# pdrebello/flash-attention-minitorch

Measured on AMD Instinct MI355X. Metric: attn fw+bw TFLOP/s at (B=8,H=8,N=4096,d=64); % MFMA roofline, higher is better.
Workload: dtype bf16

## Files before the change

flash_attention_minitorch_amd/csrc/fa_api.hip:

```cpp
#include <hip/hip_runtime.h>
#include <math.h>
#include <algorithm>
#include <chrono>
#include <mutex>
#include <string>
#include <vector>
#include <stdio.h>
#include <stdlib.h>
#include <string.h>
#include <unistd.h>
#include <atomic>

#include "../../include/flash_attn_mi355x.h"
#include "fa_kernels.h"

namespace {

thread_local char g_err[512] = "";

int set_err(int code, const char* what, hipError_t e = hipSuccess) {
  if (e != hipSuccess)
    snprintf(g_err, sizeof(g_err), "%s: %s", what, hipGetErrorString(e));
  else
    snprintf(g_err, sizeof(g_err), "%s", what);
  return code;
}

#define FA_HIP_TRY(expr)                                             \
  do {                                                               \
    hipError_t e_ = (expr);                                          \
    if (e_ != hipSuccess) return set_err(FA_ERR_HIP, #expr, e_);     \
  } while (0)

constexpr double FWD_SPLITK_MAX_WGS_PER_CU = 0.5, FWD_SPLITK_MAX_WGS_PER_CU_CAUSAL = 1.0;

inline bool d_supported(int d) { return d == 32 || d == 64 || d == 128; }
inline int d_padded(int d) { return d <= 32 ? 32 : (d <= 64 ? 64 : 128); }

constexpr int NTUN = 10;
struct Tun { int v[NTUN]; };
inline Tun default_tun() { return Tun{{0, 0, 0, 0, 0, 0, 0, 0, 0, 0}}; }
int parse_opts(const int* opts, int nopts, Tun& t) {
  t = default_tun();
  if (nopts < 0 || nopts > NTUN || (nopts > 0 && !opts)) return set_err(FA_ERR_BAD_ARG, "bad options array");
  for (int i = 0; i < nopts; ++i) t.v[i] = opts[i];
  static const int allowed[NTUN][7] = {{0, 3, 4, 5, 6, 7, -1}, {0, 2, 3, 4, -1}, {0, 2, 3, -1}, {0, -1}, {0, 1, 4, 5, -1}, {0, 1, -1}, {0, -1}, {0, 1, 2, -1},
                                       {0, 1, 2, 3, -1}, {0, 1, -1}};
  for (int i = 0; i < NTUN; ++i) {
    bool ok = false;
    for (int j = 0; allowed[i][j] >= 0; ++j) ok |= allowed[i][j] == t.v[i];
    if (!ok) return set_err(FA_ERR_BAD_ARG, "option value not supported (retired diagnostic values included)");
  }
  return FA_OK;
}

constexpr int WS_VECS = 3;

struct Call {
  const void *q = nullptr, *k = nullptr, *v = nullptr, *dout = nullptr;
  float *out = nullptr, *l = nullptr, *m = nullptr, *dq = nullptr, *dk = nullptr, *dv = nullptr, *ws = nullptr;
  bool bwd = false;
  int B = 0, H = 1;
  bool by_heads = false;
  int layout = FA_LAYOUT_BHND;
  int N = 0, d = 0;
  bool padded = false;
  int dp = 0;
  int causal = 0, variant = 0, dtype = 0;
  int stages = 0;
  const int* opts = nullptr;
  int nopts = 0;
  const float* kmask = nullptr;
  int mask_heads = 1;
  float drop_rate = 0.f, drop_scale = 1.f;
  unsigned drop_seed = 0;
  float scale = 0.f;
  bool scale_required = false;
  const float* guard = nullptr;
  int produce = 0;
  bool gqa = false;
  int Hkv = 0;
  float *gdk = nullptr, *gdv = nullptr;
  hipStream_t st = nullptr;
  int batch = 0;
  Tun tun = default_tun();
  fa::Layout lay{};
  float tau = 0.f;
  float* nlc() const { return ws; }
  float* delta() const { return ws + (long)batch * N; }
  float* nl2() const { return ws + 2 * (long)batch * N; }
};

int device_cus_raw();
int device_cus() {
  const int n = device_cus_raw();
  return n > 0 ? n : 256;
}
int device_cus_raw() {
  static std::mutex mu;
  static int cus[64];
  int dev = 0;
  if (hipGetDevice(&dev) != hipSuccess || dev < 0 || dev >= 64) return 0;
  std::lock_guard<std::mutex> lock(mu);
  if (cus[dev] == 0) {
    int n = 0;
    if (hipDeviceGetAttribute(&n, hipDeviceAttributeMultiprocessorCount, dev) != hipSuccess) return 0;
    cus[dev] = n;
  }
  return cus[dev];
}

int rank_chunk(int wgs_per_cu, int nb) {
  return std::max(1, device_cus() * wgs_per_cu / (4 * nb));
}

bool causal_ranked(const Tun& tun, int blocks, int wgs_per_cu) {
  if (tun.v[7]) return tun.v[7] == 2;
  return blocks < 8 * device_cus() * wgs_per_cu;
}

int head_tiles(const Call& c, int nb) {
  int tiles = 1;
  if (c.N % 256 == 0 && c.tun.v[5] == 0 && c.lay.G == 1) {
    const int cus = device_cus();
    for (int t = 2; t <= 16; ++t)
      if (c.batch % t == 0 && (c.batch / t) % 8 == 0 && (long)(c.batch / t) * nb >= cus) tiles = t;
  }
  return tiles;
}

inline bool guard_rows_fold(int dtype, int row_elems) { return dtype == FA_DTYPE_BF16 && (row_elems == 64 || row_elems == 128); }
int launch_scale_guard(const void* q, const void* k, long rows, long krows, int row_elems, int dtype, void* guard, hipStream_t st) {
  if (!guard_rows_fold(dtype, row_elems)) {
    FA_HIP_TRY(hipMemsetAsync(guard, 0, (size_t)2 * fa::GUARD_SLOTS * sizeof(float), st));
    return FA_OK;
  }
  const dim3 grid(fa::GUARD_SLOTS, 2);
  if (row_elems == 64)
    hipLaunchKernelGGL((fa::scale_guard_kernel<64>), grid, dim3(256), 0, st, (const fa::bf16_t*)q, (const fa::bf16_t*)k, rows, krows, (float*)guard);
  else
    hipLaunchKernelGGL((fa::scale_guard_kernel<128>), grid, dim3(256), 0, st, (const fa::bf16_t*)q, (const fa::bf16_t*)k, rows, krows, (float*)guard);
  FA_HIP_TRY(hipGetLastError());
  return FA_OK;
}

#define FA_KERNS(X)                                                                                                                  \
  X(FWD_SPLITK, "fwd_splitk_f32_kernel")                                                                                             \
  X(FWD_SLOT_CAUSAL, "fwd_slot_kernel") X(FWD_SLOT_WHOLE, "fwd_slot_kernel") X(FWD_SLOT_MASKED, "fwd_slot_kernel")                   \
  X(FWD_DROP, "fwd_kernel") X(FWD_MASK, "fwd_kernel") X(FWD_CARE, "fwd_kernel") X(FWD_MAIN, "fwd_kernel")                            \
  X(BWD_PREP, "bwd_prep_kernel")                                                                                                     \
  X(DQ_DROP, "bwd_dq_kernel") X(DQ_MASK, "bwd_dq_kernel") X(DQ_CARE, "bwd_dq_kernel") X(DQ_MAIN, "bwd_dq_kernel")                    \
  X(DQ_WAVE8, "bwd_dq_kernel")                                                                                                       \
  X(DQ_SLOT_CAUSAL, "bwd_dq_slot_kernel") X(DQ_SLOT_TILED, "bwd_dq_slot_kernel") X(DQ_SLOT_WHOLE, "bwd_dq_slot_kernel")              \
  X(DQ_SLOT_MASKED, "bwd_dq_slot_kernel")                                                                                            \
  X(DKDV_SLOT, "bwd_dkdv_slot_kernel") X(DKDV_SLOT_CAUSAL, "bwd_dkdv_slot_kernel")                                                   \
  X(DKDV_SLOT64_TILED, "bwd_dkdv_slot_kernel")            \
  X(DKDV_CARE_DROP, "bwd_dkdv_kernel") X(DKDV_CARE, "bwd_dkdv_kernel") X(DKDV_DROP_F32, "bwd_dkdv_kernel")                           \
  X(DKDV_CARE_MAIN, "bwd_dkdv_kernel") X(DKDV_PAIRED, "bwd_dkdv_kernel") X(DKDV_PAIRED_M3, "bwd_dkdv_kernel")                        \
  X(DKDV_PLAIN, "bwd_dkdv_kernel") X(DKDV_F32_64, "bwd_dkdv_kernel")                                                                 \
  X(ONEPASS, "bwd_onepass_f32_kernel")                                                                                               \
  X(GROUP_SUM, "group_sum_kernel")          \
  X(GUARD_PASS, "scale_guard_kernel")                                                        \
  X(GUARD_PASS_ZERO, nullptr)                             \
  X(GUARD_ZERO, "memset")                                                  \
  X(ZERO_GRADS, nullptr)
#define X(id, name) id,
enum Kern : int { FA_KERNS(X) };
#undef X
#define X(id, name) name,
constexpr const char* KERN_NAME[] = {FA_KERNS(X)};
#undef X
#define X(id, name) #id,
constexpr const char* BUILD_NAME[] = {FA_KERNS(X)};
#undef X

struct Step {
  Kern kern;
  unsigned grid, block;
  int nb;
  int arg;
  int rank_chunk = 0, tiles = 0, twin_blocks = 0, guard_want = 0;
  bool prep = false;
  bool check = true;
};
struct Selection {
  Step steps[8] = {};
  int n = 0;
  bool folds = false;
  bool produces_guard = false;
  bool fuses_prep = false;
  int onepass = 0;
  Step& add(Kern kern, int grid, int block, int nb = 0, int arg = 0) {
    return steps[n++] = Step{kern, (unsigned)grid, (unsigned)block, nb, arg};
  }
  void append(const Selection& o, int guard_want = 0) {
    for (int i = 0; i < o.n; ++i) (steps[n++] = o.steps[i]).guard_want = guard_want;
    folds |= o.folds;
    produces_guard |= o.produces_guard;
    fuses_prep |= o.fuses_prep;
    onepass |= o.onepass;
  }
};

void select_phased(Selection& s, const Call& c, bool bf, Kern base, int only_qb, int care_main, int ranked, bool prep) {
  const int batch = c.batch, N = c.N, causal = c.causal, nqb = (N + 127) / 128;
  const bool fwd = base == FWD_DROP;
  const int chunk = (ranked && causal && only_qb < 0) ? rank_chunk(2, nqb) : 0;
  int twin = 1;
  if (fwd && c.lay.guard && c.lay.guard_want == 1 && !causal && only_qb < 0)
    for (int t = 4; t > 1; t >>= 1)
      if (nqb % t == 0 && (long)batch * (nqb / t) >= 2L * device_cus()) { twin = t; break; }
  const int nblk = only_qb >= 0 ? 1 : ((causal && !chunk) ? (nqb + 1) / 2 : nqb / twin);
  const int build = c.lay.drop_thr ? 0
                    : c.lay.kmask  ? 1
                    : (bf && (N < 64 || only_qb >= 0 || (causal && care_main))) ? 2 : 3;
  Step& m = s.add(Kern(base + build), batch * nblk, 256, nqb, only_qb);
  m.rank_chunk = chunk;
  m.twin_blocks = fwd ? twin : 0;
  if (build != 3) return;
  m.prep = prep;
  if (bf && causal) {
    m.check = false;
    s.add(Kern(base + 2), batch, 256, nqb, 0).twin_blocks = m.twin_blocks;
  }
}

template <typename T, int D>
Selection select_fwd(const Call& c) {
  constexpr bool BF = sizeof(T) == 2;
  const int batch = c.batch, N = c.N, causal = c.causal;
  const Tun& tun = c.tun;
  const bool plain = !c.lay.kmask && !c.lay.drop_thr;
  Selection s;
  if (!BF && D == 64) {
    const long wgs = (long)batch * ((N + 127) / 128), cus = device_cus();
    if (plain && !c.lay.out_bf16 && N >= 128 && (tun.v[1] == 4 ||
         (tun.v[1] == 0 && wgs <= (causal ? FWD_SPLITK_MAX_WGS_PER_CU_CAUSAL : FWD_SPLITK_MAX_WGS_PER_CU) * cus))) {
      const int nqb = (N + 31) / 32;
      s.add(FWD_SPLITK, batch * nqb, 256, nqb);
      return s;
    }
  }
  if (BF && (D == 64 || D == 128)) {
    const int nqb = (N + 255) / 256;
    const bool cslot = causal && N % 256 == 0 && (tun.v[1] == 3 || (tun.v[1] == 0 && batch * nqb >= 256));
    if (c.variant == FA_VARIANT_FA2 && tun.v[1] != 2 && (!causal || tun.v[1] == 3 || cslot) && plain && N >= 64) {
      if (cslot) {
        const bool ranked = causal_ranked(tun, batch * nqb, D == 64 ? 2 : 1);
        s.add(FWD_SLOT_CAUSAL, ranked ? batch * nqb : batch * ((nqb + 1) / 2), 512, nqb, ranked ? 2 : 1).rank_chunk =
            rank_chunk(D == 64 ? 2 : 1, nqb);
        s.folds = true;
        return s;
      }
      if (!causal && N % (8192 / D) == 0) {
        s.add(FWD_SLOT_WHOLE, batch * nqb, 512, nqb, causal);
        s.folds = s.produces_guard = true;
        return s;
      }
      if (D == 64) {
        s.add(FWD_SLOT_MASKED, batch * nqb, 512, nqb, causal);
        if (causal) select_phased(s, c, BF, FWD_DROP, 0, 0, 0, false);
        return s;
      }
    }
  }
  select_phased(s, c, BF, FWD_DROP, -1, D == 64 ? 1 : 0, tun.v[7] == 2 || (tun.v[7] == 0 && BF && D == 32), false);
  return s;
}

template <typename T, int D>
void select_dkdv_phased(Selection& s, const Call& c, bool mode3 = false, int care_main = 0, int rank_causal = 1) {
  constexpr bool BF = sizeof(T) == 2;
  constexpr int NW = BF ? 8 : 4;
  const int batch = c.batch, N = c.N, causal = c.causal;
  const int nkb = (N + NW * 32 - 1) / (NW * 32), nkb4 = (N + 127) / 128;
  const bool rank = causal && rank_causal;
  if (c.lay.drop_thr) {
    if (BF) s.add(DKDV_CARE_DROP, batch * nkb4, 256, nkb4).rank_chunk = rank ? rank_chunk(2, nkb4) : 0;
    else s.add(DKDV_DROP_F32, batch * nkb, NW * 64, nkb).rank_chunk = rank ? rank_chunk(2, nkb) : 0;
    return;
  }
  if (BF && (c.lay.kmask || N < 64)) {
    s.add(DKDV_CARE, batch * nkb4, 256, nkb4).rank_chunk = rank ? rank_chunk(2, nkb4) : 0;
    return;
  }
  if (mode3 && causal && care_main) {
    s.add(DKDV_CARE_MAIN, batch * ((nkb + 1) / 2), NW * 64, nkb);
    return;
  }
  const int thin = (BF && causal) ? 1 : 0;
  Step* m;
  if ((causal || mode3) && !(BF && D == 128)) {
    m = &s.add(mode3 ? DKDV_PAIRED_M3 : DKDV_PAIRED, batch * ((nkb + 1) / 2), NW * 64, nkb, thin);
  } else {
    m = &s.add(DKDV_PLAIN, batch * nkb, NW * 64, nkb, thin);
    m->rank_chunk = rank ? rank_chunk(NW == 8 ? 1 : 2, nkb) : 0;
  }
  if (thin) {
    m->check = false;
    s.add(DKDV_CARE, batch, 256, nkb4, 2).rank_chunk = m->rank_chunk;
  }
}

template <typename T, int D>
int onepass_f32(const Call& c) {
  const int N = c.N;
  const Tun& tun = c.tun;
  const int both = FA_BWD_STAGE_DKDV | FA_BWD_STAGE_DQ;
  if (!(sizeof(T) == 4 && D == 64 && (c.stages & both) == both && (tun.v[4] == 0 || tun.v[4] == 5) && !c.lay.kmask &&
        !c.lay.drop_thr && N >= 256))
    return 0;
  static const bool deterministic = [] { const char* e = getenv("FA_MI355X_DETERMINISTIC"); return e && e[0] == '1'; }();
  if (deterministic && tun.v[4] != 5) return 0;
  const long cus = device_cus(), wgs1 = (long)c.batch * ((N + 255) / 256), nqi = (N + 31) / 32;
  for (int pass = (c.causal && N >= 1024) ? 0 : 1; pass < 2; ++pass)
    for (int split = 1; split <= 8; split *= 2) {
      if (split > 1 && nqi / split < 4) break;
      const long wgs = wgs1 * split, rounds = (wgs + cus - 1) / cus;
      if (pass == 0 && rounds < 2) continue;
      if (5 * wgs >= 4 * rounds * cus) return split;
    }
  return tun.v[4] == 5 ? 1 : 0;
}

bool dq64_phased(const Call& c) {
  return c.tun.v[2] == 2 || (c.causal && c.tun.v[2] != 3 && !(c.N % 256 == 0 && c.batch * (c.N / 256) >= 128));
}

template <typename T, int D>
Selection select_dq(const Call& c, bool prep) {
  constexpr bool BF = sizeof(T) == 2;
  const int batch = c.batch, N = c.N, causal = c.causal;
  Selection s;
  const bool few_keys = c.lay.kmask || c.lay.drop_thr || N < 64;
  if (BF && D == 128 && !causal && !few_keys) {
    const int nqb = (N + 255) / 256;
    s.add(DQ_WAVE8, batch * nqb, 512, nqb, -1).prep = prep;
  } else if (BF && D == 64 && !few_keys && !dq64_phased(c)) {
    const int nqb = (N + 255) / 256;
    Step* m;
    if (causal && N % 256 == 0) {
      const bool paired = !causal_ranked(c.tun, batch * nqb, 1);
      m = &s.add(DQ_SLOT_CAUSAL, paired ? batch * ((nqb + 1) / 2) : batch * nqb, 512, nqb, paired ? 1 : 2);
    } else if (!causal && N % 128 == 0) {
      const int tiles = head_tiles(c, nqb);
      m = tiles > 1 ? &s.add(DQ_SLOT_TILED, (batch / tiles) * nqb, 512, nqb, causal) : &s.add(DQ_SLOT_WHOLE, batch * nqb, 512, nqb, causal);
      m->tiles = tiles > 1 ? tiles : 0;
    } else {
      m = &s.add(DQ_SLOT_MASKED, batch * nqb, 512, nqb, causal);
      prep = false;
    }
    m->prep = prep;
    m->rank_chunk = rank_chunk(1, nqb);
    if (m->kern == DQ_SLOT_MASKED && causal) select_phased(s, c, BF, DQ_DROP, 0, 0, 0, false);
  } else {
    select_phased(s, c, BF, DQ_DROP, -1, 0, c.tun.v[7] == 2 || (c.tun.v[7] == 0 && BF && D == 32), prep);
  }
  s.fuses_prep = s.steps[0].prep;
  return s;
}

template <typename T, int D>
Selection select_dkdv(const Call& c) {
  constexpr bool BF = sizeof(T) == 2;
  const int batch = c.batch, N = c.N, causal = c.causal;
  const Tun& tun = c.tun;
  Selection s;
  if (BF && D == 64) {
    const bool plain = !c.lay.drop_thr && !c.lay.kmask;
    if (!causal && (tun.v[0] == 0 || tun.v[0] == 6 || tun.v[0] == 7) && plain && N >= 64) {
      const int nkb = (N + 255) / 256, tiles = head_tiles(c, nkb);
      const bool can64 = N % 256 == 0 && c.lay.G == 1;
      if (can64 && (tun.v[0] == 7 || (tun.v[0] == 0 && tiles > 1))) {
        const int t64 = tiles > 1 ? tiles : (c.tun.v[5] ? 1 : 4);
        s.add(DKDV_SLOT64_TILED, ((batch + t64 - 1) / t64) * nkb, 256, nkb).tiles = t64;
      } else s.add(DKDV_SLOT, batch * nkb, 512, nkb);
      return s;
    }
    if (causal && plain && N % 256 == 0 && (tun.v[0] == 5 || (tun.v[0] == 0 && batch * (N / 256) >= 128))) {
      const int nkb = N / 256;
      s.add(DKDV_SLOT_CAUSAL, batch * nkb, 512, nkb).rank_chunk = rank_chunk(1, nkb);
      return s;
    }
    if (tun.v[0] != 4) {
      select_dkdv_phased<T, D>(s, c, true, 1);
      return s;
    }
  }
  if (BF && D <= 64) {
    select_dkdv_phased<T, D>(s, c);
  } else if (BF) {
    select_dkdv_phased<T, D>(s, c, false, 0, tun.v[7] != 1);
  } else if (D == 64 && !c.lay.drop_thr) {
    const int nkb = (N + 127) / 128;
    s.add(DKDV_F32_64, batch * nkb, 256, nkb).rank_chunk = (causal && tun.v[7] != 1) ? rank_chunk(2, nkb) : 0;
  } else {
    select_dkdv_phased<T, D>(s, c);
  }
  return s;
}

template <typename T, int D>
Selection select_bwd(const Call& c) {
  const long rows = (long)c.batch * c.N;
  constexpr int RPB = 256 / (D / 8);
  const int need = FA_BWD_STAGE_PREP | FA_BWD_STAGE_DQ;
  Selection s, dq;
  s.onepass = onepass_f32<T, D>(c);
  const bool two_kernels = s.onepass && c.lay.G > 1;
  if (two_kernels) s.onepass = 0;
  if ((c.stages & FA_BWD_STAGE_DQ) && !s.onepass)
    dq = select_dq<T, D>(c, (c.stages & need) == need && c.tun.v[4] == 0 && !two_kernels);
  s.fuses_prep = dq.fuses_prep;
  if ((c.stages & FA_BWD_STAGE_PREP) && !s.fuses_prep) s.add(BWD_PREP, (int)((rows + RPB - 1) / RPB), 256);
  if (s.fuses_prep) s.append(dq);
  if (s.onepass) {
    s.add(ZERO_GRADS, 0, 0, 0, s.onepass);
    const int nkb = (c.N + 255) / 256;
    s.add(ONEPASS, c.batch * nkb * s.onepass, 512, nkb, s.onepass).rank_chunk =
        c.causal ? rank_chunk(1, nkb) : 0;
    return s;
  }
  if (c.stages & FA_BWD_STAGE_DKDV) {
    s.append(select_dkdv<T, D>(c));
    if (c.lay.G > 1) s.add(GROUP_SUM, (int)((rows / c.lay.G * (D / 4) + 255) / 256), 256);
  }
  if (!s.fuses_prep) s.append(dq);
  return s;
}

template <typename T, int D>
int execute(const Call& c, const Selection& sel) {
  constexpr bool BF = sizeof(T) == 2;
  constexpr int BN = BF ? 64 : 32, NW = BF ? 8 : 4, QS = BF ? (D == 128 ? 64 : 128) : 32;
  const int batch = c.batch, N = c.N, causal = c.causal;
  const long rows = (long)batch * N;
#define FA_GO(kern, ...) hipLaunchKernelGGL(kern, dim3(s.grid), dim3(s.block), 0, c.st, __VA_ARGS__)
#define FA_QKV (const T*)c.q, (const T*)c.k, (const T*)c.v
#define FA_FWD(FEAT, CARE) \
  FA_GO((fa::fwd_kernel<T, D, BN, 1, FEAT, CARE>), FA_QKV, c.out, c.l, c.m, N, s.nb, batch, lay, causal, c.variant, c.tau, s.arg)
#define FA_FWD_SLOT(...) FA_GO((fa::fwd_slot_kernel<__VA_ARGS__>), FA_QKV, c.out, c.l, N, s.nb, batch, lay, s.arg, c.tau)
#define FA_DQ(FEAT, NWQ, ...)                                                                                                    \
  FA_GO((fa::bwd_dq_kernel<T, D, 32, FEAT, NWQ, ##__VA_ARGS__>), FA_QKV, (const T*)c.dout, c.nlc(), c.delta(), c.dq, N, s.nb, batch, lay, \
        causal, c.tau, s.arg, pa)
#define FA_DQ_SLOT(...)                                                                                                            \
  FA_GO((fa::bwd_dq_slot_kernel<T, D, ##__VA_ARGS__>), FA_QKV, (const T*)c.dout, c.nlc(), c.delta(), c.dq, N, s.nb, batch, lay, s.arg, \
        c.tau, pa)
#define FA_DKDV_SLOT(...)                                                                                                         \
  FA_GO((fa::bwd_dkdv_slot_kernel<T, 64, ##__VA_ARGS__>), FA_QKV, (const T*)c.dout, c.nl2(), c.delta(), c.dk, c.dv, N, s.nb, batch, lay, \
        c.tau)
#define FA_DKDV(...)                                                                                                               \
  FA_GO((fa::bwd_dkdv_kernel<T, D, 32, __VA_ARGS__>), FA_QKV, (const T*)c.dout, c.nlc(), c.delta(), c.dk, c.dv, N, s.nb, batch, lay, \
        causal, c.tau, s.arg)
#define FA_ONEPASS(C, R)                                                                                                         \
  FA_GO((fa::bwd_onepass_f32_kernel<D, C, R>), FA_QKV, (const T*)c.dout, c.nlc(), c.delta(), c.dq, c.dk, c.dv, N, s.nb, batch, lay, \
        c.tau, s.arg)
  for (int i = 0; i < sel.n; ++i) {
    const Step& s = sel.steps[i];
    fa::Layout lay = c.lay;
    lay.rank_chunk = s.rank_chunk;
    lay.tiles = s.tiles;
    lay.twin_blocks = s.twin_blocks;
    lay.guard_want = s.guard_want;
    const fa::DqPrep pa = s.prep ? fa::DqPrep{c.out, c.l, c.m, c.nlc(), c.delta(), c.nl2(), c.variant, 1.0f / c.tau} : fa::DqPrep{};
    switch (s.kern) {
      case FWD_SPLITK:
        if constexpr (!BF && D == 64)
          FA_GO((fa::fwd_splitk_f32_kernel<D>), FA_QKV, c.out, c.l, c.m, N, s.nb, batch, lay, causal, c.variant, c.tau);
        break;
      case FWD_SLOT_CAUSAL:
        if constexpr (BF && D >= 64) FA_FWD_SLOT(T, D, false, 64, (D == 64 ? 4 : 2), true);
        break;
      case FWD_SLOT_WHOLE:
        if constexpr (BF && D == 64) FA_FWD_SLOT(T, 64, false, 64, 4);
        else if constexpr (BF && D == 128) FA_FWD_SLOT(T, D, false);
        break;
      case FWD_SLOT_MASKED:
        if constexpr (BF && D == 64) FA_FWD_SLOT(T, D, true);
        break;
      case FWD_DROP: FA_FWD(2, BF); break;
      case FWD_MASK: FA_FWD(1, BF); break;
      case FWD_CARE: FA_FWD(0, BF); break;
      case FWD_MAIN: FA_FWD(0, false); break;
      case BWD_PREP:
        FA_GO((fa::bwd_prep_kernel<T, D>), c.out, (const T*)c.dout, c.l, c.m, c.nlc(), c.delta(), c.nl2(), rows, N, lay, c.variant,
              1.0f / c.tau);
        break;
      case DQ_DROP: FA_DQ(2, 4, BF); break;
      case DQ_MASK: FA_DQ(1, 4, BF); break;
      case DQ_CARE: FA_DQ(0, 4, BF); break;
      case DQ_MAIN: FA_DQ(0, 4, false); break;
      case DQ_WAVE8:
        if constexpr (BF && D == 128) FA_DQ(0, 8);
        break;
      case DQ_SLOT_CAUSAL:
        if constexpr (BF && D == 64) FA_DQ_SLOT(false, true);
        break;
      case DQ_SLOT_TILED:
        if constexpr (BF && D == 64) FA_DQ_SLOT(false, false, true);
        break;
      case DQ_SLOT_WHOLE:
        if constexpr (BF && D == 64) FA_DQ_SLOT(false);
        break;
      case DQ_SLOT_MASKED:
        if constexpr (BF && D == 64) FA_DQ_SLOT();
        break;
      case DKDV_SLOT64_TILED:
        if constexpr (BF && D == 64)
          FA_GO((fa::bwd_dkdv_slot64_kernel<T, 64>), FA_QKV, (const T*)c.dout, c.nl2(), c.delta(), c.dk, c.dv, N, s.nb, batch, lay, c.tau);
        break;
      case DKDV_SLOT:
        if constexpr (BF && D == 64) FA_DKDV_SLOT();
        break;
      case DKDV_SLOT_CAUSAL:
        if constexpr (BF && D == 64) FA_DKDV_SLOT(true);
        break;
      case DKDV_CARE_DROP:
        if constexpr (BF) FA_DKDV(4, 64, 1, true, 1, BF);
        break;
      case DKDV_CARE:
        if constexpr (BF) FA_DKDV(4, 64, 1, false, 1, BF);
        break;
      case DKDV_DROP_F32:
        if constexpr (!BF) FA_DKDV(NW, QS, 1, true);
        break;
      case DKDV_CARE_MAIN:
        if constexpr (BF && D == 64) FA_DKDV(NW, QS, 3, false, 1, true, true);
        break;
      case DKDV_PAIRED:
        if constexpr (!(BF && D == 128) && !(!BF && D == 64)) FA_DKDV(NW, QS, 0, false, 1, false, true);
        break;
      case DKDV_PAIRED_M3:
        if constexpr (BF && D == 64) FA_DKDV(NW, QS, 3, false, 1, false, true);
        break;
      case DKDV_PLAIN:
        if constexpr (!(!BF && D == 64)) FA_DKDV(NW, QS, 0);
        break;
      case DKDV_F32_64:
        if constexpr (!BF && D == 64)
          FA_GO((fa::bwd_dkdv_kernel<T, D, 32, 4, 32, 0, false, 2>), FA_QKV, (const T*)c.dout, c.nlc(), c.delta(), c.dk, c.dv, N, s.nb,
                batch, lay, causal, c.tau);
        break;
      case ONEPASS:
        if constexpr (!BF && D == 64) {
          if (N % 256 == 0) {
            if (causal) FA_ONEPASS(true, false); else FA_ONEPASS(false, false);
          } else {
            if (causal) FA_ONEPASS(true, true); else FA_ONEPASS(false, true);
          }
        }
        break;
      case GROUP_SUM:
        FA_GO(fa::group_sum_kernel, c.dk, c.dv, c.gdk, c.gdv, rows / lay.G * (D / 4),
              c.layout == FA_LAYOUT_BNHD ? (long)(D / 4) : (long)N * (D / 4), lay.G);
        break;
      case GUARD_PASS:
      case GUARD_PASS_ZERO:
        if (const int rc = launch_scale_guard(c.q, c.k, rows, rows / lay.G, c.dp, c.dtype, const_cast<float*>(c.guard), c.st)) return rc;
        continue;
      case GUARD_ZERO:
        FA_HIP_TRY(hipMemsetAsync(const_cast<float*>(c.guard), 0, (size_t)2 * fa::GUARD_SLOTS * sizeof(float), c.st));
        continue;
      case ZERO_GRADS:
        FA_HIP_TRY(hipMemsetAsync(c.dq, 0, (size_t)rows * D * sizeof(float), c.st));
        if (s.arg > 1) {
          FA_HIP_TRY(hipMemsetAsync(c.dk, 0, (size_t)rows * D * sizeof(float), c.st));
          FA_HIP_TRY(hipMemsetAsync(c.dv, 0, (size_t)rows * D * sizeof(float), c.st));
        }
        continue;
    }
    if (s.check) FA_HIP_TRY(hipGetLastError());
  }
#undef FA_GO
#undef FA_QKV
#undef FA_FWD
#undef FA_FWD_SLOT
#undef FA_DQ
#undef FA_DQ_SLOT
#undef FA_DKDV_SLOT
#undef FA_DKDV
#undef FA_ONEPASS
  return FA_OK;
}

fa::Layout ungrouped(fa::Layout l) {
  l.G = 1;
  l.kvH = l.H;
  l.ldk = l.ld;
  return l;
}
fa::Layout bhnd(int N, int dp) { return ungrouped(fa::Layout{1, dp, (long)N * dp, 0, nullptr, 1, 0u, 1.0f, 0u, 0}); }
fa::Layout bnhd(int H, int N, int dp) { return ungrouped(fa::Layout{H, H * dp, (long)N * H * dp, (long)dp, nullptr, 1, 0u, 1.0f, 0u, 0}); }
inline size_t align256(size_t x) { return (x + 255) & ~(size_t)255; }

constexpr float GUARD_BUDGET = 1e-2f;
inline Call exact(Call call) {
  call.tun.v[1] = 2;
  return call;
}
template <typename T, int D>
Selection select_one(const Call& c) { return c.bwd ? select_bwd<T, D>(c) : select_fwd<T, D>(c); }

template <typename T, int D>
Selection select_call(Call& call, bool planning) {
  const float c = call.tau * fa::LOG2E;
  const int mode = call.tun.v[8], produce = call.produce;
  const float* guard = call.guard;
  fa::Layout& lay = call.lay;
  lay.scale_sel = 0;
  const Selection sel = select_one<T, D>(call);
  if (mode == 1 || fabsf(c - 1.0f) < 1e-6f) return sel;
  if (mode == 3 && planning) guard = reinterpret_cast<const float*>(16);
  lay.scale_sel = (mode == 2 || !guard) ? 1 : 2;
  if (lay.scale_sel == 2) {
    lay.guard = guard;
    lay.guard_coef = c * (0.001953125f * 0.57735027f) / GUARD_BUDGET;
  }
  const Kern pass = guard_rows_fold(call.dtype, call.dp) ? GUARD_PASS : GUARD_PASS_ZERO;
  Selection out;
  if (!sel.folds) {
    if (produce && guard && mode == 0) out.add(pass, 0, 0);
    out.append(sel, lay.scale_sel == 2 ? 3 : 0);
    return out;
  }
  if (mode == 2 || !guard) return select_one<T, D>(exact(call));
  if (produce && sel.produces_guard) out.add(GUARD_ZERO, 0, 0);
  else if (produce) out.add(pass, 0, 0);
  out.append(sel, (produce && sel.produces_guard) ? 2 : 0);
  lay.guard_want = 1;
  out.append(select_one<T, D>(exact(call)), 1);
  return out;
}

#define FA_DISPATCH(FN, ...)                                                              \
  do {                                                                                    \
    if (c.dtype == FA_DTYPE_BF16) {                                                       \
      if (c.dp == 32) return FN<fa::bf16_t, 32>(__VA_ARGS__);                             \
      if (c.dp == 64) return FN<fa::bf16_t, 64>(__VA_ARGS__);                             \
      return FN<fa::bf16_t, 128>(__VA_ARGS__);                                            \
    } else {                                                                              \
      if (c.dp == 32) return FN<float, 32>(__VA_ARGS__);                                  \
      if (c.dp == 64) return FN<float, 64>(__VA_ARGS__);                                  \
      return FN<float, 128>(__VA_ARGS__);                                                 \
    }                                                                                     \
  } while (0)
Selection select_any(Call& c, bool planning) {
  c.tau = c.scale > 0.f ? c.scale : sqrtf(1.0f / (float)c.d);
  if (!c.bwd) c.lay.out_bf16 = c.tun.v[9] == 1 ? 1 : 0;
  FA_DISPATCH(select_call, c, planning);
}
int execute_any(const Call& c, const Selection& sel) { FA_DISPATCH(execute, c, sel); }
#undef FA_DISPATCH
// ... 713 lines not shown
```

flash_attention_minitorch_amd/csrc/fa_atoms.h:

```cpp
#pragma once
#include <hip/hip_runtime.h>
#include <stdint.h>

namespace fa {

typedef __bf16 bf16_t;
typedef __attribute__((ext_vector_type(8))) __bf16 bf16x8;
typedef __attribute__((ext_vector_type(4))) __bf16 bf16x4;
typedef __attribute__((ext_vector_type(2))) __bf16 bf16x2;
typedef __attribute__((ext_vector_type(16))) float f32x16;
typedef __attribute__((ext_vector_type(8))) float f32x8;
typedef __attribute__((ext_vector_type(4))) float f32x4;
typedef __attribute__((ext_vector_type(2))) float f32x2;
typedef __attribute__((ext_vector_type(4))) uint32_t u32x4;

typedef __attribute__((address_space(3))) char lds_char;
#define FA_LDS(T, p) ((__attribute__((address_space(3))) T*)(p))
#define FA_DEV __device__ __forceinline__

FA_DEV constexpr int acc_row(int i, int h) { return (i & 3) + 8 * (i >> 2) + 4 * h; }

FA_DEV float xhalf_max(float x) {
  auto r = __builtin_amdgcn_permlane32_swap(__float_as_uint(x), __float_as_uint(x), false, false);
  return fmaxf(__uint_as_float(r[0]), __uint_as_float(r[1]));
}
FA_DEV float xhalf_sum(float x) {
  auto r = __builtin_amdgcn_permlane32_swap(__float_as_uint(x), __float_as_uint(x), false, false);
  return __uint_as_float(r[0]) + __uint_as_float(r[1]);
}

struct LaneAddr { int b[2]; };

template <typename T> struct Atom;

template <> struct Atom<bf16_t> {
  typedef bf16x8 frag;
  static constexpr int ESZ = 2;
  template <int D> static constexpr int tile_bytes(int rows) { return rows * D * 2; }
  template <int D> static FA_DEV constexpr int off(int row, int ch) {
    return (D / 32) * 512 * (row >> 3) + 512 * (ch >> 2) + 64 * (row & 7) + 16 * ((ch & 3) ^ ((row >> 2) & 3));
  }
  static FA_DEV frag zero() { frag z; for (int j = 0; j < 8; ++j) z[j] = (bf16_t)0.0f; return z; }
  static FA_DEV frag load_global(const bf16_t* p) { return *reinterpret_cast<const frag*>(p); }

  template <int D> static FA_DEV LaneAddr row_addr(int lane) {
    const int r = lane & 31, h = lane >> 5;
    LaneAddr a;
    const int rowpart = (D / 32) * 512 * (r >> 3) + 64 * (r & 7);
    a.b[0] = rowpart + 16 * ((0 + h) ^ ((r >> 2) & 3));
    a.b[1] = rowpart + 16 * ((2 + h) ^ ((r >> 2) & 3));
    return a;
  }
  template <int D> static FA_DEV frag row_frag(lds_char* tile, const LaneAddr& a, int row32, int kc) {
    return *FA_LDS(frag, tile + a.b[kc & 1] + (D / 32) * 512 * (row32 >> 3) + 512 * (kc >> 1));
  }
  template <int D> static FA_DEV LaneAddr tr_addr(int lane) {
    const int i = lane & 15, qq = i >> 2, p = i & 3, dsel = (lane >> 4) & 1, h = lane >> 5;
    LaneAddr a;
    const int c = 2 * dsel + (p >> 1);
    a.b[0] = 64 * (4 * h + qq) + 16 * (c ^ h) + 8 * (p & 1);
    a.b[1] = 64 * (4 * h + qq) + 16 * (c ^ (h + 2)) + 8 * (p & 1);
    return a;
  }
  template <int D> static FA_DEV frag tr_frag(lds_char* tile, const LaneAddr& a, int rowbase, int ct) {
    const int k = (D / 32) * 512 * (rowbase >> 3) + 512 * ct;
    bf16x4 lo = __builtin_amdgcn_ds_read_tr16_b64_v4bf16(FA_LDS(bf16x4, tile + a.b[0] + k));
    bf16x4 hi = __builtin_amdgcn_ds_read_tr16_b64_v4bf16(FA_LDS(bf16x4, tile + a.b[1] + k + (D / 32) * 512));
    return __builtin_shufflevector(lo, hi, 0, 1, 2, 3, 4, 5, 6, 7);
  }
  static FA_DEV frag pack(const f32x16& x, int s) {
    typedef __attribute__((ext_vector_type(4))) uint32_t u4;
    u4 u;
#pragma unroll
    for (int j = 0; j < 4; ++j) {
      f32x2 pr = {x[8 * s + 2 * j], x[8 * s + 2 * j + 1]};
      u[j] = __builtin_bit_cast(uint32_t, __builtin_convertvector(pr, bf16x2));
    }
    return __builtin_bit_cast(frag, u);
  }
  static FA_DEV frag pack_lo(const f32x16& x, int s, const frag& hi) {
    typedef __attribute__((ext_vector_type(4))) uint32_t u4;
    const u4 hu = __builtin_bit_cast(u4, hi);
    u4 u;
#pragma unroll
    for (int j = 0; j < 4; ++j) {
      const float h0 = __uint_as_float(hu[j] << 16), h1 = __uint_as_float(hu[j] & 0xffff0000u);
      f32x2 pr = {x[8 * s + 2 * j] - h0, x[8 * s + 2 * j + 1] - h1};
      u[j] = __builtin_bit_cast(uint32_t, __builtin_convertvector(pr, bf16x2));
    }
    return __builtin_bit_cast(frag, u);
  }
  static constexpr bool SPLITS = true;
  static FA_DEV frag scale(const frag& a, float c) {
    frag o;
#pragma unroll
    for (int j = 0; j < 8; ++j) o[j] = (bf16_t)((float)a[j] * c);
    return o;
  }
  static FA_DEV void mma(f32x16& acc, const frag& a, const frag& b) {
    acc = __builtin_amdgcn_mfma_f32_32x32x16_bf16(a, b, acc, 0, 0, 0);
  }
  static FA_DEV void mma_c(f32x16& d, const frag& a, const frag& b, const f32x16& c0) {
    d = __builtin_amdgcn_mfma_f32_32x32x16_bf16(a, b, c0, 0, 0, 0);
  }
};

struct MfmaRC {
  typedef bf16x8 frag;
  static FA_DEV void ag(f32x16& acc, const frag& a, const frag& b) {
    asm volatile("v_mfma_f32_32x32x16_bf16 %0, %1, %2, %0" : "+a"(acc) : "v"(a), "v"(b));
  }
  static FA_DEV void ag_z(f32x16& acc, const frag& a, const frag& b) {
    asm volatile("s_nop 1\n\tv_mfma_f32_32x32x16_bf16 %0, %1, %2, 0" : "=a"(acc) : "v"(a), "v"(b));
  }
  static FA_DEV void vs(f32x16& d, const frag& a, const frag& b_agpr) {
    asm volatile("v_mfma_f32_32x32x16_bf16 %0, %1, %2, %0" : "+v"(d) : "v"(a), "a"(b_agpr));
  }
  static FA_DEV void vs_c(f32x16& d, const frag& a, const frag& b_agpr, const f32x16& c0) {
    asm volatile("v_mfma_f32_32x32x16_bf16 %0, %1, %2, %3" : "=&v"(d) : "v"(a), "a"(b_agpr), "v"(c0));
  }
  static FA_DEV frag to_agpr(const frag& x) {
    frag y;
    asm volatile("s_nop 1" : "=a"(y) : "0"(x));
    return y;
  }
  static FA_DEV void mma_drain(f32x16 (&x)[2][2], f32x16 (&y)[2][2]) {
    asm volatile("s_nop 15\n\ts_nop 15"
                 : "+a"(x[0][0]), "+a"(x[0][1]), "+a"(x[1][0]), "+a"(x[1][1]), "+a"(y[0][0]), "+a"(y[0][1]), "+a"(y[1][0]), "+a"(y[1][1]));
  }
};

template <> struct Atom<float> {
  typedef f32x8 frag;
  static constexpr int ESZ = 4;
  template <int D> static constexpr int tile_bytes(int rows) { return rows * (D + 4) * 4; }
  template <int D> static FA_DEV constexpr int off(int row, int ch) { return row * (D + 4) * 4 + ch * 16; }
  static FA_DEV frag zero() { frag z; for (int j = 0; j < 8; ++j) z[j] = 0.0f; return z; }
  static FA_DEV frag load_global(const float* p) {
    f32x4 a = *reinterpret_cast<const f32x4*>(p);
    f32x4 b = *reinterpret_cast<const f32x4*>(p + 4);
    return __builtin_shufflevector(a, b, 0, 1, 2, 3, 4, 5, 6, 7);
  }
  template <int D> static FA_DEV LaneAddr row_addr(int lane) {
    const int r = lane & 31, h = lane >> 5;
    LaneAddr a;
    a.b[0] = a.b[1] = (r * (D + 4) + 8 * h) * 4;
    return a;
  }
  template <int D> static FA_DEV frag row_frag(lds_char* tile, const LaneAddr& a, int row32, int kc) {
    const int k = (row32 * (D + 4) + 16 * kc) * 4;
    f32x4 x = *FA_LDS(f32x4, tile + a.b[0] + k);
    f32x4 y = *FA_LDS(f32x4, tile + a.b[0] + k + 16);
    return __builtin_shufflevector(x, y, 0, 1, 2, 3, 4, 5, 6, 7);
  }
  template <int D> static FA_DEV LaneAddr tr_addr(int lane) {
    const int r = lane & 31, h = lane >> 5;
    LaneAddr a;
    a.b[0] = a.b[1] = (4 * h * (D + 4) + r) * 4;
    return a;
  }
  template <int D> static FA_DEV frag tr_frag(lds_char* tile, const LaneAddr& a, int rowbase, int ct) {
    frag f;
#pragma unroll
    for (int j = 0; j < 8; ++j)
      f[j] = *FA_LDS(float, tile + a.b[0] + ((rowbase + 8 * (j >> 2) + (j & 3)) * (D + 4) + 32 * ct) * 4);
    return f;
  }
  static FA_DEV frag pack(const f32x16& x, int s) {
    frag f;
#pragma unroll
    for (int j = 0; j < 8; ++j) f[j] = x[8 * s + j];
    return f;
  }
  static FA_DEV frag pack_lo(const f32x16&, int, const frag&) { return zero(); }
  static constexpr bool SPLITS = false;
  static FA_DEV frag scale(const frag& a, float c) {
    frag o;
#pragma unroll
    for (int j = 0; j < 8; ++j) o[j] = a[j] * c;
    return o;
  }
  static FA_DEV void mma(f32x16& acc, const frag& a, const frag& b) {
#pragma unroll
    for (int j = 0; j < 8; ++j) acc = __builtin_amdgcn_mfma_f32_32x32x2f32(a[j], b[j], acc, 0, 0, 0);
  }
  static FA_DEV void mma_c(f32x16& d, const frag& a, const frag& b, const f32x16& c0) {
    d = __builtin_amdgcn_mfma_f32_32x32x2f32(a[0], b[0], c0, 0, 0, 0);
#pragma unroll
    for (int j = 1; j < 8; ++j) d = __builtin_amdgcn_mfma_f32_32x32x2f32(a[j], b[j], d, 0, 0, 0);
  }
};

typedef __amdgpu_buffer_rsrc_t rsrc_t;
FA_DEV rsrc_t make_rsrc(const void* p, uint32_t bytes) {
  return __builtin_amdgcn_make_buffer_rsrc(const_cast<void*>(p), 0, bytes, 0x00020000);
}

typedef u32x4 raw_rsrc_t;
FA_DEV raw_rsrc_t make_raw_rsrc(const void* p, uint32_t bytes) {
  const uint64_t a = (uint64_t)p;
  raw_rsrc_t r = {(uint32_t)a, (uint32_t)(a >> 32) & 0xffffu, bytes, 0x00020000u};
  return r;
}
FA_DEV void dma16(raw_rsrc_t rs, uint32_t lds_dst, int voff, int soff) {
  uint32_t keep;
  asm volatile(
      "s_mov_b32 %0, m0\n\ts_mov_b32 m0, %1\n\ts_nop 0\n\tbuffer_load_dwordx4 %2, %3, %4 offen lds\n\ts_mov_b32 m0, %0"
      : "=&s"(keep)
      : "s"(lds_dst), "v"(voff), "s"(rs), "s"(soff)
      : "memory");
}
FA_DEV void dma4(raw_rsrc_t rs, uint32_t lds_dst, int voff, int soff) {
  uint32_t keep;
  asm volatile(
      "s_mov_b32 %0, m0\n\ts_mov_b32 m0, %1\n\ts_nop 0\n\tbuffer_load_dword %2, %3, %4 offen lds\n\ts_mov_b32 m0, %0"
      : "=&s"(keep)
      : "s"(lds_dst), "v"(voff), "s"(rs), "s"(soff)
      : "memory");
}
FA_DEV void dma_wait_all() { asm volatile("s_waitcnt vmcnt(0)" ::: "memory"); }

#define FA_DMA_VOFF(name, PPG, lane, w, ld, esz)                              \
  const int dma_row7 = ((lane) >> 2) & 7;                                     \
  const int dma_gpar = ((PPG) == 1) ? ((w) & 1) : (((w) >> 1) & 1);           \
  const int dma_half = ((PPG) == 1) ? 0 : ((w) & 1);                          \
  const int name = dma_row7 * (ld) * (esz) +                                  \
                   16 * (4 * (2 * dma_half + ((lane) >> 5)) + (((lane) & 3) ^ ((2 * dma_gpar + (dma_row7 >> 2)) & 3)))

template <int D, int ROWS, int NW = 8>
struct StageRing {
  using A = Atom<bf16_t>;
  typedef A::frag frag;
  static constexpr int PPG = D / 64;
  static constexpr int NPW = A::tile_bytes<D>(ROWS) / 1024 / NW;
  static constexpr int SUBB = (D / 32) * 512 * 4;
  static_assert((D == 64 || D == 128) && A::tile_bytes<D>(ROWS) % (1024 * NW) == 0 && NW % 4 == 0,
                "every wave moves whole pieces of one swizzle parity");
  static constexpr bool dma_matches_image() {
    constexpr int LDB = 1 << 16;
    for (int w = 0; w < NW; ++w)
      for (int i = 0; i < NPW; ++i)
        for (int lane = 0; lane < 64; ++lane) {
          FA_DMA_VOFF(so, PPG, lane, w, LDB / A::ESZ, A::ESZ);
          const int piece = w + NW * i, row = 8 * (piece / PPG) + so / LDB, ch = so % LDB / 16;
          if (so % 16 != 0 || ch >= D / 8 || A::off<D>(row, ch) != 1024 * piece + 16 * lane) return false;
        }
    return true;
  }
  static FA_DEV frag row(lds_char* smem, int b0, int b1, int sub, int kc, int toff = 0) {
    return *FA_LDS(frag, smem + ((kc & 1) ? b1 : b0) + toff + SUBB * sub + 512 * (kc >> 1));
  }
  static FA_DEV frag tr(lds_char* smem, int b0, int b1, int sub, int s2, int dt, int toff = 0) {
    const int kk = toff + SUBB * sub + (D / 32) * 512 * (2 * s2) + 512 * dt;
    bf16x4 lo = __builtin_amdgcn_ds_read_tr16_b64_v4bf16(FA_LDS(bf16x4, smem + b0 + kk));
    bf16x4 hi = __builtin_amdgcn_ds_read_tr16_b64_v4bf16(FA_LDS(bf16x4, smem + b1 + kk + (D / 32) * 512));
    return __builtin_shufflevector(lo, hi, 0, 1, 2, 3, 4, 5, 6, 7);
  }
};
template <int R, int SLOTB> FA_DEV constexpr int ring_slot(int st, int roff = 0) { return ((st + roff) % R) * SLOTB; }

template <typename T, int D, int ROWS, int NT> struct TileStager {
  static constexpr int CPR = D * (int)sizeof(T) / 16;
  static constexpr int NCH = ROWS * CPR;
  static constexpr int PER = (NCH + NT - 1) / NT;
  static constexpr int RSTEP = NT / CPR;
  static_assert(NT % CPR == 0, "threads must tile whole rows");
  static_assert(sizeof(T) == 4 || RSTEP % 16 == 0 || PER == 1, "row step must keep the swizzle phase");
  u32x4 regs[PER];
  int voff;
  int lds_off;
  int ldb;
  bool live;
  FA_DEV void init(int tid, int ld) {
    ldb = ld * (int)sizeof(T);
    int row = tid / CPR, ch = tid % CPR;
    if constexpr (sizeof(T) == 2 && CPR >= 8) {
      const int g = tid >> 3;
      row = 2 * (g / (CPR / 4)) + ((tid >> 2) & 1);
      ch = 4 * (g % (CPR / 4)) + (tid & 3);
    }
    voff = row * ldb + ch * 16;
// ... 95 lines not shown
```

flash_attention_minitorch_amd/csrc/fa_kernels.h:

```cpp
#pragma once
#include "fa_common.h"
#include "fa_fwd.h"
#include "fa_fwd_splitk_f32.h"
#include "fa_bwd_dkdv.h"
#include "fa_bwd_dkdv64.h"
#include "fa_bwd_dq.h"
#include "fa_bwd_onepass_f32.h"
#include "fa_aux.h"
```

Measured before the change: 942.3.

## Add 4-wave d=64 dQ slot kernel with multi-head tiling for non-causal backward

```diff
diff --git a/flash_attention_minitorch_amd/csrc/fa_api.hip b/flash_attention_minitorch_amd/csrc/fa_api.hip
--- a/flash_attention_minitorch_amd/csrc/fa_api.hip
+++ b/flash_attention_minitorch_amd/csrc/fa_api.hip
@@ -44,7 +44,7 @@
   t = default_tun();
   if (nopts < 0 || nopts > NTUN || (nopts > 0 && !opts)) return set_err(FA_ERR_BAD_ARG, "bad options array");
   for (int i = 0; i < nopts; ++i) t.v[i] = opts[i];
-  static const int allowed[NTUN][7] = {{0, 3, 4, 5, 6, 7, -1}, {0, 2, 3, 4, -1}, {0, 2, 3, -1}, {0, -1}, {0, 1, 4, 5, -1}, {0, 1, -1}, {0, -1}, {0, 1, 2, -1},
+  static const int allowed[NTUN][7] = {{0, 3, 4, 5, 6, 7, -1}, {0, 2, 3, 4, -1}, {0, 2, 3, 6, 7, -1}, {0, -1}, {0, 1, 4, 5, -1}, {0, 1, -1}, {0, -1}, {0, 1, 2, -1},
                                        {0, 1, 2, 3, -1}, {0, 1, -1}};
   for (int i = 0; i < NTUN; ++i) {
     bool ok = false;
@@ -151,7 +151,8 @@
   X(BWD_PREP, "bwd_prep_kernel")                                                                                                     \
   X(DQ_DROP, "bwd_dq_kernel") X(DQ_MASK, "bwd_dq_kernel") X(DQ_CARE, "bwd_dq_kernel") X(DQ_MAIN, "bwd_dq_kernel")                    \
   X(DQ_WAVE8, "bwd_dq_kernel")                                                                                                       \
-  X(DQ_SLOT_CAUSAL, "bwd_dq_slot_kernel") X(DQ_SLOT_TILED, "bwd_dq_slot_kernel") X(DQ_SLOT_WHOLE, "bwd_dq_slot_kernel")              \
+  X(DQ_SLOT_CAUSAL, "bwd_dq_slot_kernel") X(DQ_SLOT_WHOLE, "bwd_dq_slot_kernel")                                                     \
+  X(DQ_SLOT_TILED, "bwd_dq_slot_kernel")                 \
   X(DQ_SLOT_MASKED, "bwd_dq_slot_kernel")                                                                                            \
   X(DKDV_SLOT, "bwd_dkdv_slot_kernel") X(DKDV_SLOT_CAUSAL, "bwd_dkdv_slot_kernel")                                                   \
   X(DKDV_SLOT64_TILED, "bwd_dkdv_slot_kernel")            \
@@ -344,8 +345,12 @@
       m = &s.add(DQ_SLOT_CAUSAL, paired ? batch * ((nqb + 1) / 2) : batch * nqb, 512, nqb, paired ? 1 : 2);
     } else if (!causal && N % 128 == 0) {
       const int tiles = head_tiles(c, nqb);
-      m = tiles > 1 ? &s.add(DQ_SLOT_TILED, (batch / tiles) * nqb, 512, nqb, causal) : &s.add(DQ_SLOT_WHOLE, batch * nqb, 512, nqb, causal);
-      m->tiles = tiles > 1 ? tiles : 0;
+      const bool can64 = N % 256 == 0 && c.lay.G == 1;
+      if (can64 && (c.tun.v[2] == 7 || (c.tun.v[2] != 6 && tiles > 1))) {
+        const int t64 = tiles > 1 ? tiles : (c.tun.v[5] ? 1 : 4);
+        m = &s.add(DQ_SLOT_TILED, ((batch + t64 - 1) / t64) * nqb, 256, nqb, causal);
+        m->tiles = t64;
+      } else m = &s.add(DQ_SLOT_WHOLE, batch * nqb, 512, nqb, causal);
     } else {
       m = &s.add(DQ_SLOT_MASKED, batch * nqb, 512, nqb, causal);
       prep = false;
@@ -497,7 +502,8 @@
         if constexpr (BF && D == 64) FA_DQ_SLOT(false, true);
         break;
       case DQ_SLOT_TILED:
-        if constexpr (BF && D == 64) FA_DQ_SLOT(false, false, true);
+        if constexpr (BF && D == 64)
+          FA_GO((fa::bwd_dq_slot64_kernel<T, 64>), FA_QKV, (const T*)c.dout, c.nlc(), c.delta(), c.dq, N, s.nb, batch, lay, c.tau, pa);
         break;
       case DQ_SLOT_WHOLE:
         if constexpr (BF && D == 64) FA_DQ_SLOT(false);
diff --git a/flash_attention_minitorch_amd/csrc/fa_atoms.h b/flash_attention_minitorch_amd/csrc/fa_atoms.h
--- a/flash_attention_minitorch_amd/csrc/fa_atoms.h
+++ b/flash_attention_minitorch_amd/csrc/fa_atoms.h
@@ -127,6 +127,9 @@
   static FA_DEV void mma_drain(f32x16 (&x)[2][2], f32x16 (&y)[2][2]) {
     asm volatile("s_nop 15\n\ts_nop 15"
                  : "+a"(x[0][0]), "+a"(x[0][1]), "+a"(x[1][0]), "+a"(x[1][1]), "+a"(y[0][0]), "+a"(y[0][1]), "+a"(y[1][0]), "+a"(y[1][1]));
+  }
+  static FA_DEV void mma_drain(f32x16 (&x)[2][2]) {
+    asm volatile("s_nop 15\n\ts_nop 15" : "+a"(x[0][0]), "+a"(x[0][1]), "+a"(x[1][0]), "+a"(x[1][1]));
   }
 };
 
diff --git a/flash_attention_minitorch_amd/csrc/fa_bwd_dq64.h b/flash_attention_minitorch_amd/csrc/fa_bwd_dq64.h
--- /dev/null
+++ b/flash_attention_minitorch_amd/csrc/fa_bwd_dq64.h
@@ -0,0 +1,250 @@
+#pragma once
+#include "fa_common.h"
+#include "fa_bwd_dq.h"
+
+namespace fa {
+
+template <typename T, int D>
+__global__ void __launch_bounds__(256) __attribute__((amdgpu_waves_per_eu(1, 1)))
+bwd_dq_slot64_kernel(const T* __restrict__ q, const T* __restrict__ k, const T* __restrict__ v, const T* __restrict__ dout,
+                     const float* __restrict__ nlc, const float* __restrict__ ndelta, float* __restrict__ dq, int N, int nqb,
+                     int BH, Layout lay, float tau, DqPrep pa = DqPrep{}) {
+  if (guard_skip(lay)) return;
+  static_assert(D == 64 && sizeof(T) == 2, "slot schedule is laid out for bf16, d = 64");
+  using A = Atom<T>;
+  using M = MfmaRC;
+  typedef typename A::frag frag;
+  constexpr int KC = 4, ST = 128, NW = 4, QG = 2, QPW = 32 * QG, BQ = NW * QPW;
+  constexpr int TB = A::template tile_bytes<D>(ST);
+  constexpr int VOFF = 3 * TB;
+  using RG = StageRing<D, ST, NW>;
+  static_assert(RG::dma_matches_image() && RG::NPW == 4, "LDS-DMA source swizzle vs Atom::off");
+  __shared__ __attribute__((aligned(16))) char smem_raw[6 * TB];
+  lds_char* smem = (lds_char*)smem_raw;
+
+  const int tid = threadIdx.x, lane = tid & 63, r = lane & 31, h = lane >> 5;
+  const int w = __builtin_amdgcn_readfirstlane(tid >> 6);
+  const int tiles = max(lay.tiles, 1);
+  int bh, qb;
+  map_block(blockIdx.x, (BH + tiles - 1) / tiles, nqb, bh, qb);
+  bh *= tiles;
+  const int heads = min(tiles, BH - bh);
+  size_t base = head_base(lay, bh);
+  const int ld = lay.ld;
+  const uint32_t mat_bytes = ((uint32_t)(N - 1) * ld + D) * (uint32_t)sizeof(T);
+  rsrc_t qrs = make_rsrc(q + base, mat_bytes), dors = make_rsrc(dout + base, mat_bytes);
+  raw_rsrc_t kraw = make_raw_rsrc(k + base, mat_bytes), vraw = make_raw_rsrc(v + base, mat_bytes);
+  const float c = tau * LOG2E;
+  const bool exact = scale_exact(lay);
+  const int qw0 = qb * BQ + w * QPW;
+
+  frag ql[QG][KC], dl[QG][KC];
+  float nlq[QG], ndq[QG];
+  auto load_q = [&]() {
+#pragma unroll
+    for (int g = 0; g < QG; ++g)
+#pragma unroll
+      for (int kc = 0; kc < KC; ++kc) {
+        const int off = ((qw0 + 32 * g + r) * ld + 16 * kc + 8 * h) * (int)sizeof(T);
+        ql[g][kc] = load_frag_buf<T>(qrs, off);
+        dl[g][kc] = load_frag_buf<T>(dors, off);
+      }
+#pragma unroll
+    for (int g = 0; g < QG; ++g) {
+      const int qrow = qw0 + 32 * g + r;
+      if (pa.o != nullptr) {
+        dq_prep_rows<T, KC>(pa, dl[g], base, bh, N, qrow, ld, h, true, c, nlq[g], ndq[g]);
+      } else {
+        nlq[g] = nlc[(size_t)bh * N + qrow] * c;
+        ndq[g] = ndelta[(size_t)bh * N + qrow];
+      }
+    }
+  };
+
+  const LaneAddr ra = A::template row_addr<D>(lane);
+  const LaneAddr ta = A::template tr_addr<D>(lane);
+  const int nstage = N / ST;
+  const uint32_t smem_addr = (uint32_t)(uintptr_t)smem;
+  FA_DMA_VOFF(dma_voff, RG::PPG, lane, w, ld, (int)sizeof(T));
+  auto stage_dma = [&](int row0, int slot_base) {
+#pragma unroll
+    for (int i = 0; i < RG::NPW; ++i) {
+      const int g = w + NW * i;
+      const int soff = (row0 + 8 * g) * ld * (int)sizeof(T);
+      dma16(kraw, smem_addr + slot_base + 1024 * g, dma_voff, soff);
+      dma16(vraw, smem_addr + slot_base + VOFF + 1024 * g, dma_voff, soff);
+    }
+  };
+
+  auto sweep = [&](auto ex_c) {
+  constexpr bool EX = decltype(ex_c)::value != 0;
+  frag qa[QG][KC], da[QG][KC];
+  f32x16 acc[QG][2];
+  f32x16 sA[QG], dpA[QG], sB[QG], dpB[QG], nl16[QG], nd16[QG];
+  frag dsA0[QG], dsA1[QG], dsB0[QG], dsB1[QG];
+  frag F[4];
+  int cb = 0, tb = 0;
+  int R0 = ra.b[0], R1 = ra.b[1], T0 = ta.b[0], T1 = ta.b[1];
+  auto SB = [&]() { __builtin_amdgcn_sched_barrier(0); };
+  auto period = [&](auto hn_c, auto hc_c, auto hp_c, auto first_c, auto updr_c, auto updt_c, auto subn_c, auto subp_c, auto sub2_c,
+                    int dr, int dtb, f32x16(&ns)[QG], f32x16(&ndp)[QG], f32x16(&cs)[QG], f32x16(&cdp)[QG], frag(&dp0)[QG],
+                    frag(&dp1)[QG], frag(&dc0)[QG], frag(&dc1)[QG]) {
+    constexpr bool HN = decltype(hn_c)::value != 0, HC = decltype(hc_c)::value != 0, HP = decltype(hp_c)::value != 0;
+    constexpr bool FIRST = decltype(first_c)::value != 0, UPDR = decltype(updr_c)::value != 0, UPDT = decltype(updt_c)::value != 0;
+    constexpr int SUBN = decltype(subn_c)::value, SUBP = decltype(subp_c)::value, SUB2 = decltype(sub2_c)::value;
+    auto fe = [&](int g, int i) { cs[g][i] = EX ? __builtin_amdgcn_exp2f(cs[g][i] * c) : __builtin_amdgcn_exp2f(cs[g][i]); };
+    auto md = [&](int g, int i) { cdp[g][i] = cs[g][i] * cdp[g][i]; };
+#pragma unroll
+    for (int s = 0; s < 24; ++s) {
+      const int kk = s >> 1, g = s & 1, kq = kk & 3;
+      if (kk < 4) {
+        if constexpr (HN) {
+          if (kq == 0) M::vs_c(ns[g], F[0], qa[g][0], nl16[g]);
+          else M::vs(ns[g], F[kq], qa[g][kq]);
+          SB();
+        }
+      } else if (kk < 8) {
+        if constexpr (HN) {
+          if (kq == 0) M::vs_c(ndp[g], F[0], da[g][0], nd16[g]);
+          else M::vs(ndp[g], F[kq], da[g][kq]);
+          SB();
+        }
+      } else {
+        if constexpr (HP) {
+          M::ag(acc[g][kq & 1], F[kq], (kq < 2) ? dp0[g] : dp1[g]);
+          SB();
+        }
+      }
+      if (g == 0) {
+        const int f = (kk + 3) & 3;
+        if (s == 0) {
+          if constexpr (HN && !FIRST) F[3] = RG::row(smem, R0, R1, SUBN, 3);
+        } else if (s <= 8) {
+          if constexpr (HN) F[f] = RG::row(smem, R0, R1, SUBN, f, VOFF);
+        } else if (s <= 16) {
+          if constexpr (HP) F[f] = RG::tr(smem, T0, T1, SUBP, f >> 1, f & 1);
+        } else {
+          if constexpr (HN) F[f] = RG::row(smem, R0, R1, SUB2, f);
+        }
+      }
+      if constexpr (UPDR) {
+        if (s == 9) { R0 += dr; R1 += dr; }
+      }
+      if constexpr (UPDT) {
+        if (s == 17) { T0 += dtb; T1 += dtb; }
+      }
+      if constexpr (HC) {
+        if (s < 16) { fe(g, 2 * kk); fe(g, 2 * kk + 1); }
+        switch (s) {
+          case 1: md(0, 0); md(0, 1); break;
+          case 2: md(1, 0); break;
+          case 3: md(1, 1); md(0, 2); break;
+          case 4: md(0, 3); break;
+          case 5: md(1, 2); md(1, 3); break;
+          case 6: md(0, 4); break;
+          case 7: md(0, 5); md(1, 4); break;
+          case 8: md(1, 5); break;
+          case 9: md(0, 6); md(0, 7); break;
+          case 11: md(1, 6); md(1, 7); break;
+          case 13: md(0, 8); md(0, 9); break;
+          case 15: md(1, 8); md(1, 9); break;
+          case 16: dc0[0] = A::pack(cdp[0], 0); break;
+          case 17: dc0[1] = A::pack(cdp[1], 0); md(0, 10); md(0, 11); break;
+          case 18: md(1, 10); md(1, 11); md(0, 12); md(0, 13); md(1, 12); break;
+          case 19: md(1, 13); md(0, 14); md(0, 15); md(1, 14); md(1, 15); break;
+          case 20: dc1[0] = A::pack(cdp[0], 1); break;
+          case 21: dc1[1] = A::pack(cdp[1], 1); break;
+          default: break;
+        }
+      }
+      SB();
+    }
+  };
+  auto install = [&]() {
+#pragma unroll
+    for (int g = 0; g < QG; ++g)
+#pragma unroll
+      for (int kc = 0; kc < KC; ++kc) {
+        qa[g][kc] = M::to_agpr(EX ? ql[g][kc] : A::scale(ql[g][kc], c));
+        da[g][kc] = M::to_agpr(dl[g][kc]);
+      }
+#pragma unroll
+    for (int g = 0; g < QG; ++g)
+#pragma unroll
+      for (int i = 0; i < 16; ++i) {
+        nd16[g][i] = ndq[g];
+        nl16[g][i] = EX ? nlq[g] * (1.0f / c) : nlq[g];
+      }
+    asm volatile("s_nop 1" : "+v"(nl16[0]), "+v"(nl16[1]), "+v"(nd16[0]), "+v"(nd16[1]));
+    const frag z = A::zero();
+#pragma unroll
+    for (int g = 0; g < QG; ++g)
+#pragma unroll
+      for (int dt = 0; dt < 2; ++dt) M::ag_z(acc[g][dt], z, z);
+  };
+  stage_dma(0, 0);
+  load_q();
+  install();
+  dma_wait_all();
+  __syncthreads();
+  auto T1_ = ic<1>{};
+  auto T0_ = ic<0>{};
+  for (int t = 0; t < heads; ++t) {
+  T0 += cb - tb; T1 += cb - tb;
+  tb = cb;
+#pragma unroll
+  for (int kc = 0; kc < 4; ++kc) F[kc] = RG::row(smem, R0, R1, 0, kc);
+#pragma unroll
+  for (int g = 0; g < QG; ++g) {
+    dsB0[g] = A::zero();
+    dsB1[g] = A::zero();
+  }
+  SB();
+  period(T1_, T0_, T0_, T1_, T0_, T0_, ic<0>{}, ic<0>{}, ic<1>{}, 0, 0, sA, dpA, sB, dpB, dsB0, dsB1, dsA0, dsA1);
+  for (int st = 0; st < nstage; ++st) {
+    const int nb = (cb == 2 * TB) ? 0 : cb + TB;
+    if (st + 1 < nstage) stage_dma((st + 1) * ST, nb);
+    else if (t + 1 < heads) {
+      const size_t nbase = head_base(lay, bh + 1);
+      kraw = make_raw_rsrc(k + nbase, mat_bytes);
+      vraw = make_raw_rsrc(v + nbase, mat_bytes);
+      stage_dma(0, nb);
+    }
+    period(T1_, T1_, T1_, T0_, T0_, T1_, ic<1>{}, ic<3>{}, ic<2>{}, 0, cb - tb, sB, dpB, sA, dpA, dsB0, dsB1, dsA0, dsA1);
+    tb = cb;
+    period(T1_, T1_, T1_, T0_, T0_, T0_, ic<2>{}, ic<0>{}, ic<3>{}, 0, 0, sA, dpA, sB, dpB, dsA0, dsA1, dsB0, dsB1);
+    dma_wait_all();
+    __syncthreads();
+    period(T1_, T1_, T1_, T0_, T1_, T0_, ic<3>{}, ic<1>{}, ic<0>{}, nb - cb, 0, sB, dpB, sA, dpA, dsB0, dsB1, dsA0, dsA1);
+    cb = nb;
+    period(T1_, T1_, T1_, T0_, T0_, T0_, ic<0>{}, ic<2>{}, ic<1>{}, 0, 0, sA, dpA, sB, dpB, dsA0, dsA1, dsB0, dsB1);
+  }
+  period(T0_, T0_, T1_, T0_, T0_, T0_, ic<0>{}, ic<3>{}, ic<0>{}, 0, 0, sB, dpB, sA, dpA, dsB0, dsB1, dsA0, dsA1);
+  float* dqrow = dq + base + (size_t)(qw0 + r) * ld;
+  if (t + 1 < heads) {
+    ++bh;
+    base = head_base(lay, bh);
+    qrs = make_rsrc(q + base, mat_bytes);
+    dors = make_rsrc(dout + base, mat_bytes);
+    load_q();
+  }
+  M::mma_drain(acc);
+#pragma unroll
+  for (int g2 = 0; g2 < QG; ++g2)
+#pragma unroll
+    for (int dt = 0; dt < 2; ++dt) {
+      const f32x16 x = acc[g2][dt];
+#pragma unroll
+      for (int g = 0; g < 4; ++g) {
+        f32x4 val = {x[4 * g] * tau, x[4 * g + 1] * tau, x[4 * g + 2] * tau, x[4 * g + 3] * tau};
+        *reinterpret_cast<f32x4*>(dqrow + (size_t)32 * g2 * ld + 32 * dt + 8 * g + 4 * h) = val;
+      }
+    }
+  if (t + 1 < heads) install();
+  }
+  };
+  if (exact) sweep(ic<1>{});
+  else sweep(ic<0>{});
+}
+
+}
diff --git a/flash_attention_minitorch_amd/csrc/fa_kernels.h b/flash_attention_minitorch_amd/csrc/fa_kernels.h
--- a/flash_attention_minitorch_amd/csrc/fa_kernels.h
+++ b/flash_attention_minitorch_amd/csrc/fa_kernels.h
@@ -5,5 +5,6 @@
 #include "fa_bwd_dkdv.h"
 #include "fa_bwd_dkdv64.h"
 #include "fa_bwd_dq.h"
+#include "fa_bwd_dq64.h"
 #include "fa_bwd_onepass_f32.h"
 #include "fa_aux.h"
```

Result: no change. 949.5, median of 6 (+0.8%).
